# dnjulek/vapoursynth-zip

Measured on AMD Instinct MI355X. Metric: frames/sec at 4K YUV420P16: Bilateral, BoxBlur, SSIMULACRA2 on 1/2/4/8 MI355X, higher is better.
Workload: dtype u16; 1 GPU; vszip.BoxBlur hradius=vradius=13, 3840x2160 YUV420P16, splitmix64 noise, HBM-resident; parallelism=frame-parallel x1, arena_candidates=9

## Files before the change

### vapoursynth-zip_amd/csrc/boxblur_ct.hpp

```cpp
#pragma once
#include <cmath>
#include <cstdlib>
#include <utility>

#include "plane_table.hpp"

namespace {

#ifndef VSZIP_ST_AUX
#define VSZIP_ST_AUX 2
#endif
#ifndef VSZIP_LD_AUX
#define VSZIP_LD_AUX 0
#endif
#ifndef VSZIP_ST8_AUX
#define VSZIP_ST8_AUX 0
#endif
#ifndef VSZIP_ST16_AUX
#define VSZIP_ST16_AUX 2
#endif
constexpr int kStoreAux = VSZIP_ST_AUX, kLoadAux = VSZIP_LD_AUX, kStoreAux8 = VSZIP_ST8_AUX, kStoreAux16 = VSZIP_ST16_AUX;
typedef uint32_t U32x4 __attribute__((ext_vector_type(4)));
typedef uint32_t U32x2 __attribute__((ext_vector_type(2)));

constexpr int kMaxPlanes = 48;
constexpr int PX = 8;

struct BBPlane {
    const void *src;
    void *dst;
    int sstride, dstride;
    int w, h;
    int block0;
    int ntx;
    int nbands;
    int nperiods;
    int cx0;
};

struct BBParams {
    BBPlane p[kMaxPlanes];
    int nplanes;
    int band_rows;
    int nblocks;
};

constexpr int kRingMaxPlanes = 192;
constexpr int kRingMaxBlocks = 8192;
struct RingParams {
    BBPlane p[kRingMaxPlanes];
    int nplanes;
    int nblocks;
    uint8_t plane_of_block[kRingMaxBlocks];
};

__device__ __forceinline__ int ct_tap_row(int k, int i, int radius, int ih) {
    const int dist_from_bottom = ih - 1 - i;
    if (k < radius) return (i < radius - k) ? min(radius - k - i, ih - 1) : (i - radius + k);
    return (dist_from_bottom < k - radius) ? (i - min(k - radius - dist_from_bottom, i)) : (i - radius + k);
}

template <typename T>
struct Raw8;
template <>
struct Raw8<uint16_t> {
    uint4 q;
};
template <>
struct Raw8<uint8_t> {
    uint2 q;
};

__device__ __forceinline__ void unpack8(const Raw8<uint16_t> &r, uint32_t v[PX]) {
    v[0] = r.q.x & 0xffffu; v[1] = r.q.x >> 16;
    v[2] = r.q.y & 0xffffu; v[3] = r.q.y >> 16;
    v[4] = r.q.z & 0xffffu; v[5] = r.q.z >> 16;
    v[6] = r.q.w & 0xffffu; v[7] = r.q.w >> 16;
}

__device__ __forceinline__ void unpack8(const Raw8<uint8_t> &r, uint32_t v[PX]) {
    v[0] = r.q.x & 0xffu; v[1] = (r.q.x >> 8) & 0xffu; v[2] = (r.q.x >> 16) & 0xffu; v[3] = r.q.x >> 24;
    v[4] = r.q.y & 0xffu; v[5] = (r.q.y >> 8) & 0xffu; v[6] = (r.q.y >> 16) & 0xffu; v[7] = r.q.y >> 24;
}

__device__ __forceinline__ void pack8(const uint32_t v[PX], Raw8<uint16_t> &r) {
    r.q.x = v[0] | (v[1] << 16);
    r.q.y = v[2] | (v[3] << 16);
    r.q.z = v[4] | (v[5] << 16);
    r.q.w = v[6] | (v[7] << 16);
}

__device__ __forceinline__ void pack8(const uint32_t v[PX], Raw8<uint8_t> &r) {
    r.q.x = v[0] | (v[1] << 8) | (v[2] << 16) | (v[3] << 24);
    r.q.y = v[4] | (v[5] << 8) | (v[6] << 16) | (v[7] << 24);
}

template <typename T, int PXN>
struct RawN : Raw8<T> {};
template <>
struct RawN<uint8_t, 16> {
    uint4 q;
};
template <typename T>
__device__ __forceinline__ void unpackN(const RawN<T, 8> &r, uint32_t v[8]) {
    unpack8(static_cast<const Raw8<T> &>(r), v);
}
__device__ __forceinline__ void unpackN(const RawN<uint8_t, 16> &r, uint32_t v[16]) {
    const uint32_t dw[4] = {r.q.x, r.q.y, r.q.z, r.q.w};
#pragma unroll
    for (int k = 0; k < 16; ++k) v[k] = (dw[k >> 2] >> (8 * (k & 3))) & 0xffu;
}

__device__ __forceinline__ int mirror_col(int c, int w) {
    c = c < 0 ? -c - 1 : c;
    c = c >= w ? 2 * w - 1 - c : c;
    return min(max(c, 0), w - 1);
}

template <typename T>
__device__ __forceinline__ Raw8<T> load8(const T *row, int vx0, int w, bool fast) {
    Raw8<T> r;
    if (fast) {
        r.q = *reinterpret_cast<const decltype(r.q) *>(row + vx0);
    } else {
        uint32_t v[PX];
#pragma unroll
        for (int k = 0; k < PX; ++k) v[k] = row[mirror_col(vx0 + k, w)];
        pack8(v, r);
    }
    return r;
}

template <typename T>
__device__ __forceinline__ void store8(T *row, int x0, int w, bool fast, const uint32_t o[PX]);

template <>
__device__ __forceinline__ void store8<uint16_t>(uint16_t *row, int x0, int w, bool fast, const uint32_t o[PX]) {
    if (fast) {
        uint4 q;
        q.x = (o[0] & 0xffffu) | (o[1] << 16);
        q.y = (o[2] & 0xffffu) | (o[3] << 16);
        q.z = (o[4] & 0xffffu) | (o[5] << 16);
        q.w = (o[6] & 0xffffu) | (o[7] << 16);
        *reinterpret_cast<uint4 *>(row + x0) = q;
    } else {
#pragma unroll
        for (int k = 0; k < PX; ++k)
            if (x0 + k < w) row[x0 + k] = (uint16_t)o[k];
    }
}

template <>
__device__ __forceinline__ void store8<uint8_t>(uint8_t *row, int x0, int w, bool fast, const uint32_t o[PX]) {
    if (fast) {
        uint2 q;
        q.x = (o[0] & 0xffu) | ((o[1] & 0xffu) << 8) | ((o[2] & 0xffu) << 16) | (o[3] << 24);
        q.y = (o[4] & 0xffu) | ((o[5] & 0xffu) << 8) | ((o[6] & 0xffu) << 16) | (o[7] << 24);
        *reinterpret_cast<uint2 *>(row + x0) = q;
    } else {
#pragma unroll
        for (int k = 0; k < PX; ++k)
            if (x0 + k < w) row[x0 + k] = (uint8_t)o[k];
    }
}

template <int R>
struct CtGeom {
    static constexpr int K = 2 * R + 1;
    static constexpr int NE = (R + 1 + PX - 1) / PX;
    static constexpr int HL = NE * PX;
    static constexpr int HR = ((R + PX - 1) / PX) * PX;
    static constexpr int OUT_LANES = 64 - NE - HL / PX - HR / PX;
    static constexpr int TWO = OUT_LANES * PX;
};

__device__ __forceinline__ void wave_lds_fence() {
    __builtin_amdgcn_fence(__ATOMIC_RELEASE, "wavefront");
    __builtin_amdgcn_wave_barrier();
    __builtin_amdgcn_fence(__ATOMIC_ACQUIRE, "wavefront");
}

template <typename T, int R, bool DPP>
__global__ __launch_bounds__(64) void boxblur_ct_int_kernel(const BBParams prm) {
    using G = CtGeom<R>;
    constexpr uint32_t K = G::K;
    constexpr uint32_t MAGIC = (uint32_t)(((1ull << 32) + K - 1) / K);
    constexpr uint64_t INV = ((1ull << 32) + R) / K;
    constexpr uint32_t INV2 = (uint32_t)(INV >> 16);
    constexpr uint32_t INVLO = (uint32_t)(INV & 0xffffu);

    __shared__ __attribute__((aligned(16))) uint32_t P[64 * PX];

    const int b = blockIdx.x;
    const BBPlane pl = prm.p[vszip_find_plane(prm, b)];
    const int lb = b - pl.block0;
    const int tx = lb % pl.ntx;
    const int by = lb / pl.ntx;
    const int w = pl.w, h = pl.h;
    const int y0 = by * prm.band_rows;
    const int y1 = min(y0 + prm.band_rows, h);
    const T *src = static_cast<const T *>(pl.src);
    T *dst = static_cast<T *>(pl.dst);

    const int lane = threadIdx.x;
    const int X0 = tx * G::TWO;
    const int vx0 = lane < G::NE ? lane * PX : X0 - G::HL + (lane - G::NE) * PX;
    constexpr int VB = sizeof(T) * PX;
    const bool src_al = ((reinterpret_cast<uintptr_t>(src) | (uintptr_t)((size_t)pl.sstride * sizeof(T))) & (VB - 1)) == 0;
    const bool dst_al = ((reinterpret_cast<uintptr_t>(dst) | (uintptr_t)((size_t)pl.dstride * sizeof(T))) & (VB - 1)) == 0;
    const bool in_fast = src_al && vx0 >= 0 && vx0 + PX <= w;
    const bool is_out = lane >= G::NE + G::HL / PX && lane < G::NE + G::HL / PX + G::OUT_LANES && vx0 < w;
    const bool out_fast = dst_al && vx0 + PX <= w;

    uint32_t col[PX];
#pragma unroll
    for (int k = 0; k < PX; ++k) col[k] = 0;
#pragma unroll 1
    for (int k = 0; k < (int)K; ++k) {
        uint32_t v[PX];
        unpack8(load8<T>(src + (size_t)ct_tap_row(k, y0, R, h) * pl.sstride, vx0, w, in_fast), v);
#pragma unroll
        for (int j = 0; j < PX; ++j) col[j] += v[j];
    }

    const int ci = lane * PX;
#pragma unroll 1
    for (int i = y0; i < y1; ++i) {
        Raw8<T> an, sn;
        const bool more = i + 1 < y1;
        if (more) {
            const int n = i + 1;
            const int ar = (n + R < h) ? n + R : n - 1;
            const int sr = (n <= R) ? R - n + 1 : n - R - 1;
            an = load8<T>(src + (size_t)ar * pl.sstride, vx0, w, in_fast);
            sn = load8<T>(src + (size_t)sr * pl.sstride, vx0, w, in_fast);
        }

        uint32_t p[PX];
#pragma unroll
        for (int k = 0; k < PX; ++k) p[k] = __umulhi(col[k] + R, MAGIC);
#pragma unroll
        for (int k = 1; k < PX; ++k) p[k] += p[k - 1];
        const uint32_t incl = DPP ? wave_incl_scan_dpp(p[PX - 1]) : wave_incl_scan_shfl(p[PX - 1]);
        const uint32_t base = incl - p[PX - 1];
#pragma unroll
        for (int k = 0; k < PX; ++k) p[k] += base;
        *reinterpret_cast<uint4 *>(&P[ci]) = make_uint4(p[0], p[1], p[2], p[3]);
        *reinterpret_cast<uint4 *>(&P[ci + 4]) = make_uint4(p[4], p[5], p[6], p[7]);
        wave_lds_fence();

        if (is_out) {
            const uint32_t e0 = P[R] + P[R - 1];
            const uint32_t krow = 32768u + (uint32_t)(((uint64_t)e0 * INVLO) >> 16);
            uint32_t o[PX];
#pragma unroll
            for (int k = 0; k < PX; ++k) {
                const uint32_t e = P[ci + k + R] - P[ci + k - R - 1];
                o[k] = (uint32_t)(((uint64_t)e * INV2 + krow) >> 16);
            }
            store8<T>(dst + (size_t)i * pl.dstride, vx0, w, out_fast, o);
        }
        wave_lds_fence();

        if (more) {
            uint32_t a[PX], sb[PX];
            unpack8(an, a);
            unpack8(sn, sb);
#pragma unroll
            for (int k = 0; k < PX; ++k) col[k] += a[k] - sb[k];
        }
    }
}



template <int R, int SLOT_VGPRS = 4, int PXN = 8, int RV = R>
struct RingGeom {
    static constexpr int K = 2 * RV + 1;
    static constexpr int HL = ((R + 1 + PXN - 1) / PXN) * PXN;
    static constexpr int HR = ((R + PXN - 1) / PXN) * PXN;
#ifdef VSZIP_RING_OUT_LANES
    static constexpr int OUT_LANES = VSZIP_RING_OUT_LANES < 64 - HL / PXN - HR / PXN ? VSZIP_RING_OUT_LANES : 64 - HL / PXN - HR / PXN;
#else
    static constexpr int OUT_LANES = 64 - HL / PXN - HR / PXN;
#endif
    static constexpr int TWO = OUT_LANES * PXN;
    static constexpr int est_vgprs(int d) { return (2 * RV + 1 + d) * SLOT_VGPRS + (PXN == 16 ? 104 : 56); }
    static constexpr int tier(int v) { return v <= 128 ? 4 : (v <= 168 ? 3 : 2); }
    static constexpr int D3 = (2 * RV + 4) % 3 == 0 ? 3 : ((2 * RV + 6) % 3 == 0 ? 5 : 7);
#ifdef VSZIP_RING_D
    static constexpr int D = VSZIP_RING_D | 1;
    static constexpr int KL = (2 * RV + 1 + D) % 3 == 0 ? 3 : 2;
#else
    static constexpr bool SHALLOW = tier(est_vgprs(1)) > tier(est_vgprs(D3));
    static constexpr int D = SHALLOW ? 1 : D3;
    static constexpr int KL = SHALLOW ? 2 : 3;
#endif
    static constexpr int NR = 2 * RV + 1 + D;
#ifdef VSZIP_RING_WPE
    static constexpr int WPE = VSZIP_RING_WPE;
#else
    static constexpr int WPE = (SLOT_VGPRS == 2 && PXN == 8) ? (tier(est_vgprs(D)) > 3 ? 3 : tier(est_vgprs(D))) : tier(est_vgprs(D));
#endif
    static_assert(NR % KL == 0, "K-column ring must divide the period");
    static constexpr uint32_t MAGIC = K > 1 ? (uint32_t)(((1ull << 32) + K - 1) / K) : 0u;
};

template <typename T, int R, bool GENERAL, int PXN = 8, bool HONLY = false>
struct RingWave {
    static_assert(PXN == 8 || (PXN == 16 && sizeof(T) == 1 && !GENERAL), "16 pixels a lane: 8-bit planes, whole 16-pixel groups");
    static constexpr int RV = HONLY ? 0 : R;
    using G = RingGeom<R, (int)(sizeof(T) * PXN / 4), PXN, RV>;
    using RawT = RawN<T, PXN>;
    using Vec = decltype(RawT{}.q);
    static constexpr int NR = G::NR;
    static constexpr uint64_t INV = ((1ull << 32) + R) / (uint64_t)(2 * R + 1);
    static constexpr uint32_t INV2 = (uint32_t)(INV >> 16);

    RawT ring[NR];
    uint32_t col[PXN];
    uint32_t kcol;
    uint32_t kwgt;
    uint32_t kvo;
    uint32_t kn[G::KL], ko[G::KL];
    uint32_t kn_off, ko_off;
    uint32_t kr_prev;
    uint32_t *P;
    const char *srcb;
    char *dstb;
    uint32_t coff;
    uint32_t doff;
    uint32_t next_off;
    uint32_t out_off;
    uint32_t srow, drow;
    int w, h, lane, c0;
    bool rev, ld_ok, is_out, out_full;
    bool plain;
    __amdgpu_buffer_rsrc_t rs, rd;
    uint32_t sdoff;
    uint32_t psel;
    static constexpr uint32_t kOOB = 0xfffffff0u;

    __device__ __forceinline__ RawT fetch_off(uint32_t row_off) const {
        RawT t;
        if constexpr (sizeof(T) * PXN == 16) {
            const auto v = __builtin_amdgcn_raw_buffer_load_b128(rs, coff, row_off, sizeof(T) == 2 ? kLoadAux : 0);
            t.q = make_uint4(v[0], v[1], v[2], v[3]);
        } else {
            const auto v = __builtin_amdgcn_raw_buffer_load_b64(rs, coff, row_off, 0);
            t.q = make_uint2(v[0], v[1]);
        }
        return t;
    }
    __device__ __forceinline__ uint32_t fetch_px(uint32_t row_off) const {
        if constexpr (sizeof(T) == 2)
            return __builtin_amdgcn_raw_buffer_load_b16(rs, kvo, row_off, 0);
        else
            return __builtin_amdgcn_raw_buffer_load_b8(rs, kvo, row_off, 0);
    }
    __device__ __forceinline__ uint32_t krow_now() const {
        constexpr uint32_t INVLO = (uint32_t)(INV & 0xffffu);
        uint32_t v = __umul24(G::K > 1 ? __umulhi(kcol, G::MAGIC) : kcol, kwgt);
        v += (uint32_t)__builtin_amdgcn_update_dpp(0, (int)v, 0x111, 0xf, 0xf, false);
        v += (uint32_t)__builtin_amdgcn_update_dpp(0, (int)v, 0x112, 0xf, 0xf, false);
        v += (uint32_t)__builtin_amdgcn_update_dpp(0, (int)v, 0x114, 0xf, 0xf, false);
        v += (uint32_t)__builtin_amdgcn_update_dpp(0, (int)v, 0x118, 0xf, 0xf, false);
        uint32_t e0;
        if constexpr (R < 16) {
            e0 = (uint32_t)__builtin_amdgcn_readlane((int)v, 15);
        } else {
            v += (uint32_t)__builtin_amdgcn_update_dpp(0, (int)v, 0x142, 0xa, 0xf, false);
            e0 = (uint32_t)__builtin_amdgcn_readlane((int)v, 31);
        }
        return 32768u + (uint32_t)(((uint64_t)e0 * INVLO) >> 16);
    }

    __device__ __forceinline__ void fix_order(RawT &r) const {
        if constexpr (GENERAL) return;
        if constexpr (sizeof(T) * PXN == 16) {
            const uint4 o = r.q;
            r.q.x = __builtin_amdgcn_perm(o.w, o.x, psel);
            r.q.y = __builtin_amdgcn_perm(o.z, o.y, psel);
            r.q.z = __builtin_amdgcn_perm(o.y, o.z, psel);
            r.q.w = __builtin_amdgcn_perm(o.x, o.w, psel);
        } else {
            const uint2 o = r.q;
            r.q.x = __builtin_amdgcn_perm(o.y, o.x, psel);
            r.q.y = __builtin_amdgcn_perm(o.x, o.y, psel);
        }
    }
    __device__ __forceinline__ uint32_t row_off(int v) const {
        const int r = v < 0 ? -v : (v < h ? v : v - RV - 1);
        return (uint32_t)min(r, h - 1) * srow;
    }

    template <int J>
    __device__ __forceinline__ void fill(int y0) {
        ring[J] = fetch_off(row_off(y0 - RV + J));
    }
    template <int J>
    __device__ __forceinline__ void accum() {
        uint32_t v[PXN];
        fix_order(ring[J]);
        unpackN(ring[J], v);
#pragma unroll
        for (int k = 0; k < PXN; ++k) col[k] += v[k];
    }
    template <int... J>
    __device__ __forceinline__ void fill_all(int y0, std::integer_sequence<int, J...>) {
        (fill<(J + G::K) % NR>(y0), ...);
    }
    template <int... J>
    __device__ __forceinline__ void accum_all(std::integer_sequence<int, J...>) {
        (accum<J>(), ...);
    }

    static __device__ __forceinline__ int pidx(int c) { return (c & (PXN - 1)) * 64 + c / PXN; }

    __device__ __forceinline__ void window_sums(const uint32_t *Pb, uint32_t e[PXN]) const {
        if constexpr (!GENERAL) {
#pragma unroll
            for (int k = 0; k < PXN; ++k) {
                const int hi = k + R, lo = k - R - 1;
                const int hi_px = hi & (PXN - 1), hi_ln = hi / PXN;
                const int lo_px = lo & (PXN - 1), lo_ln = (lo - lo_px) / PXN;
                e[k] = Pb[hi_px * 64 + lane + hi_ln] - Pb[lo_px * 64 + lane + lo_ln];
            }
        } else {
            const int off = lane * PXN - c0;
            auto lds = [&](int idx) { return Pb[pidx(min(max(idx, 0), 64 * PXN - 1))]; };
            const uint32_t qw = lds(w - 1 + off);
#pragma unroll
            for (int k = 0; k < PXN; ++k) {
                const int x = c0 + k;
                const int lo = x - R - 1, ml = R - x - 1;
                uint32_t v = lds(min(x + R, w - 1) + off) + qw - lds(min(2 * w - 2 - x - R, w - 1) + off);
                v -= lo >= 0 ? lds(lo + off) : 0u;
                v += ml >= 0 ? lds(ml + off) : 0u;
                e[k] = v;
            }
        }
    }

    __device__ __forceinline__ void emit_row(const uint32_t e[PXN], uint32_t row_off_bytes, uint32_t kr, bool live) const {
        if constexpr (GENERAL) {
            if (!live || !is_out) return;
        }
        uint32_t t[PXN];
#pragma unroll
        for (int k = 0; k < PXN; ++k) t[k] = __umul24(e[k], INV2) + kr;
        if constexpr (!GENERAL) {
#ifdef VSZIP_DIAG_NO_STORE
            const uint32_t vo = (live && lane == 8) ? sdoff : kOOB;
#else
            const uint32_t vo = live ? sdoff : kOOB;
#endif
            if constexpr (sizeof(T) == 2) {
                U32x4 v;
                v.x = __builtin_amdgcn_perm(t[1], t[0], 0x07060302u);
                v.y = __builtin_amdgcn_perm(t[3], t[2], 0x07060302u);
                v.z = __builtin_amdgcn_perm(t[5], t[4], 0x07060302u);
                v.w = __builtin_amdgcn_perm(t[7], t[6], 0x07060302u);
                __builtin_amdgcn_raw_buffer_store_b128(v, rd, vo, row_off_bytes, kStoreAux);
            } else if constexpr (PXN == 16) {
                uint32_t dw[4];
#pragma unroll
                for (int g = 0; g < 4; ++g) {
                    const uint32_t a0 = __builtin_amdgcn_perm(t[4 * g + 1], t[4 * g], 0x0c0c0602u);
                    const uint32_t a1 = __builtin_amdgcn_perm(t[4 * g + 3], t[4 * g + 2], 0x0c0c0602u);
                    dw[g] = a0 | (a1 << 16);
                }
                U32x4 v;
                v.x = dw[0];
                v.y = dw[1];
                v.z = dw[2];
                v.w = dw[3];
                __builtin_amdgcn_raw_buffer_store_b128(v, rd, vo, row_off_bytes, kStoreAux16);
            } else {
                U32x2 v;
                const uint32_t a0 = __builtin_amdgcn_perm(t[1], t[0], 0x0c0c0602u);
                const uint32_t a1 = __builtin_amdgcn_perm(t[3], t[2], 0x0c0c0602u);
                const uint32_t a2 = __builtin_amdgcn_perm(t[5], t[4], 0x0c0c0602u);
                const uint32_t a3 = __builtin_amdgcn_perm(t[7], t[6], 0x0c0c0602u);
                v.x = a0 | (a1 << 16);
                v.y = a2 | (a3 << 16);
                __builtin_amdgcn_raw_buffer_store_b64(v, rd, vo, row_off_bytes, kStoreAux8);
            }
        } else {
            T *q = reinterpret_cast<T *>(dstb + (row_off_bytes + doff));
            if (out_full) {
                if constexpr (sizeof(T) == 2) {
                    uint4 v;
                    v.x = __builtin_amdgcn_perm(t[1], t[0], 0x07060302u);
                    v.y = __builtin_amdgcn_perm(t[3], t[2], 0x07060302u);
                    v.z = __builtin_amdgcn_perm(t[5], t[4], 0x07060302u);
                    v.w = __builtin_amdgcn_perm(t[7], t[6], 0x07060302u);
                    *reinterpret_cast<uint4 *>(q) = v;
                } else {
                    uint2 v;
                    const uint32_t a0 = __builtin_amdgcn_perm(t[1], t[0], 0x0c0c0602u);
                    const uint32_t a1 = __builtin_amdgcn_perm(t[3], t[2], 0x0c0c0602u);
                    const uint32_t a2 = __builtin_amdgcn_perm(t[5], t[4], 0x0c0c0602u);
                    const uint32_t a3 = __builtin_amdgcn_perm(t[7], t[6], 0x0c0c0602u);
                    v.x = a0 | (a1 << 16);
                    v.y = a2 | (a3 << 16);
                    *reinterpret_cast<uint2 *>(q) = v;
                }
            } else {
#pragma unroll
                for (int k = 0; k < PXN; ++k)
                    if (c0 + k < w) q[k] = (T)(t[k] >> 16);
            }
        }
    }

    template <int S>
    __device__ __forceinline__ void step(int i, int y0) {
        uint32_t *Pa = P + (S & 1) * (64 * PXN);
        const uint32_t *Pb = P + ((S & 1) ^ 1) * (64 * PXN);
        __builtin_amdgcn_sched_barrier(0);

        uint32_t e[PXN];
        const bool have_prev = S > 0 || i > y0;
#ifdef VSZIP_DIAG_NO_HORIZONTAL
#pragma unroll
        for (int k = 0; k < PXN; ++k) e[k] = col[k];
#else
        if (!GENERAL || have_prev) window_sums(Pb, e);
#endif

        uint32_t p[PXN];
#pragma unroll
        for (int k = 0; k < PXN; ++k) {
            if constexpr (G::K == 1) {
                p[k] = col[k];
            } else if constexpr (sizeof(T) == 1) {
                constexpr uint32_t M19 = (uint32_t)(((1u << 19) + G::K - 1) / G::K);
                static_assert((uint64_t)(255u * G::K + RV) * (M19 * G::K - (1u << 19)) < (1u << 19), "8-bit divide-by-k shortcut must be exact");
                p[k] = __umul24(col[k], M19) >> 19;
            } else {
                p[k] = __umulhi(col[k], G::MAGIC);
            }
        }
        if constexpr (GENERAL) {
            const uint32_t m = ld_ok ? 0xffffffffu : 0u;
#pragma unroll
            for (int k = 0; k < PXN; ++k) p[k] &= m;
        }
#ifdef VSZIP_DIAG_NO_HORIZONTAL
        (void)Pa;
        kr_prev += p[0] + p[7];
#else
#pragma unroll
        for (int k = 1; k < PXN; ++k) p[k] += p[k - 1];
        const uint32_t incl = wave_incl_scan_dpp(p[PXN - 1]);
        const uint32_t base = incl - p[PXN - 1];
#pragma unroll
        for (int k = 0; k < PXN; ++k) Pa[k * 64 + lane] = p[k] + base;
#endif

        {
            constexpr int E = (S + 1 + 2 * RV) % NR;
            uint32_t a[PXN], sb[PXN];
            fix_order(ring[E]);
            unpackN(ring[E], a);
            unpackN(ring[S], sb);
#pragma unroll
            for (int k = 0; k < PXN; ++k) col[k] += a[k] - sb[k];
#ifdef VSZIP_DIAG_NO_LOAD
            if (next_off == 0xffffffffu) ring[S] = fetch_off(next_off);
#else
            ring[S] = fetch_off(next_off);
#endif

        }
        const uint32_t kr_cur = krow_now();
        {
            constexpr int J = S % G::KL;
            kcol += kn[J] - ko[J];
#ifndef VSZIP_DIAG_NO_KCOL
            kn[J] = fetch_px(kn_off);
            ko[J] = fetch_px(ko_off);
#endif

        }

        emit_row(e, out_off, kr_prev, have_prev);
        out_off += have_prev ? drow : 0u;
        kr_prev = kr_cur;
        if (plain) {
            next_off += srow;
            kn_off += srow;
            ko_off += srow;
        } else {
            next_off = row_off(i + 2 + RV + G::D);
            kn_off = row_off(i + 2 + RV + G::KL);
            ko_off = row_off(i + 1 - RV + G::KL);
        }
#ifndef VSZIP_DIAG_NO_FENCE
        wave_lds_fence();
#endif
    }

    template <int... S>
    __device__ __forceinline__ void period(int i0, int y0, std::integer_sequence<int, S...>) {
        (step<S>(i0 + S, y0), ...);
    }
};

template <typename T, int R, bool GENERAL, int PXN = 8, bool HONLY = false>
__global__ __launch_bounds__(64, (GENERAL ? 2 : RingGeom<R, (int)(sizeof(T) * PXN / 4), PXN, (HONLY ? 0 : R)>::WPE)) void boxblur_ct_ring_kernel(const RingParams prm) {
    using W = RingWave<T, R, GENERAL, PXN, HONLY>;
    using G = typename W::G;
    constexpr int RV = W::RV;
    static_assert(G::NR % 2 == 0 && G::NR <= 64, "ring period must be even and fit a wave");
    __shared__ __attribute__((aligned(16))) uint32_t P[2 * 64 * PXN];

    const int chunk = (prm.nblocks + 7) >> 3;
    const int b = (int)(blockIdx.x & 7) * chunk + (int)(blockIdx.x >> 3);
    if (b >= prm.nblocks) return;
    const int pi = prm.plane_of_block[b];
    const BBPlane pl = prm.p[pi];
    const int lb = b - pl.block0;
    const int tx = lb % pl.ntx;
    const int by = lb / pl.ntx;
    const int p0 = (int)((long)by * pl.nperiods / pl.nbands);
    const int p1 = (int)((long)(by + 1) * pl.nperiods / pl.nbands);
    const int band_rows = (p1 - p0) * G::NR;
    const int y0 = min(p0 * G::NR, pl.h - band_rows);
    const int w = pl.w;

    W st;
    st.P = P;
    st.w = w;
    st.h = pl.h;
    st.srow = (uint32_t)pl.sstride * (uint32_t)sizeof(T);
    st.drow = (uint32_t)pl.dstride * (uint32_t)sizeof(T);
    st.srcb = static_cast<const char *>(pl.src);
    st.dstb = static_cast<char *>(pl.dst);
    const int lane = threadIdx.x;
    st.lane = lane;
    const int vc0 = pl.cx0 + tx * G::TWO - G::HL + lane * PXN;
    st.c0 = vc0;
    st.is_out = lane >= G::HL / PXN && lane < G::HL / PXN + G::OUT_LANES && vc0 < w;
    st.doff = (uint32_t)(max(vc0, 0) * (int)sizeof(T));
    st.out_full = vc0 + PXN <= w;
    if constexpr (!GENERAL) {
        int g = vc0;
        st.rev = false;
        if (vc0 < 0) {
            g = -vc0 - PXN;
            st.rev = true;
        } else if (vc0 >= w) {
            g = 2 * w - vc0 - PXN;
            st.rev = true;
        }
        g = min(max(g, 0), w - PXN);
        st.coff = (uint32_t)(g * (int)sizeof(T));
        st.ld_ok = true;
    } else {
        st.rev = false;
        st.ld_ok = vc0 >= 0 && vc0 < w;
        st.coff = (uint32_t)(min(max(vc0, 0), ((w - 1) / PXN) * PXN) * (int)sizeof(T));
    }

    st.psel = st.rev ? (sizeof(T) == 2 ? 0x05040706u : 0x04050607u) : 0x03020100u;
    st.sdoff = st.is_out ? st.doff : W::kOOB;
    st.rs = __builtin_amdgcn_make_buffer_rsrc(const_cast<void *>(pl.src), 0, (int)((uint32_t)pl.h * st.srow), 0x00020000);
    st.rd = __builtin_amdgcn_make_buffer_rsrc(pl.dst, 0, (int)((uint32_t)pl.h * st.drow), 0x00020000);
    st.plain = (y0 - RV >= 0) && (y0 + band_rows + RV + G::D + 2 < pl.h);

    st.fill_all(y0, std::make_integer_sequence<int, G::NR>{});
#pragma unroll
    for (int k = 0; k < PXN; ++k) st.col[k] = RV;
    st.accum_all(std::make_integer_sequence<int, (int)G::K>{});
    {
        const int kc = min(lane, R);
        st.kvo = (uint32_t)(kc * (int)sizeof(T));
        st.kwgt = lane < R ? 2u : (lane == R ? 1u : 0u);
        uint32_t acc = RV;
#pragma unroll
        for (int k = 0; k < (int)G::K; ++k) acc += st.fetch_px(st.row_off(y0 - RV + k));
        st.kcol = acc;
#pragma unroll
        for (int j = 0; j < G::KL; ++j) {
            st.kn[j] = st.fetch_px(st.row_off(y0 + j + 1 + RV));
            st.ko[j] = st.fetch_px(st.row_off(y0 + j - RV));
        }
        st.kn_off = st.row_off(y0 + G::KL + 1 + RV);
        st.ko_off = st.row_off(y0 + G::KL - RV);
        st.kr_prev = 0;
    }
    st.next_off = st.row_off(y0 + 1 + RV + G::D);
    st.out_off = (uint32_t)y0 * st.drow;

    const int y1 = y0 + band_rows;
#pragma unroll 1
    for (int i0 = y0; i0 < y1; i0 += G::NR) st.period(i0, y0, std::make_integer_sequence<int, G::NR>{});
    {
        uint32_t e[PXN];
        st.window_sums(P + 64 * PXN, e);
        st.emit_row(e, st.out_off, st.kr_prev, true);
    }
}


template <typename T, int R>
int launch_ct_int(vszip_ctx *ctx, const vszip_plane *planes, int nplanes) {
    using G = CtGeom<R>;
    int done = 0;
    while (done < nplanes) {
        BBParams prm;
        const int n = std::min(kMaxPlanes, nplanes - done);
        prm.nplanes = n;
        long total_px = 0;
        for (int i = 0; i < n; ++i) total_px += (long)planes[done + i].w * planes[done + i].h;
        int band = 64;
        while (band > 16 && total_px / ((long)G::TWO * band) < 4096) band >>= 1;
        prm.band_rows = band;
        int blocks = 0;
        for (int i = 0; i < n; ++i) {
            const vszip_plane &s = planes[done + i];
            BBPlane &d = prm.p[i];
            d.src = s.src;
            d.dst = s.dst;
            d.sstride = (int)s.src_stride;
            d.dstride = (int)s.dst_stride;
            d.w = s.w;
            d.h = s.h;
            d.block0 = blocks;
            d.ntx = (s.w + G::TWO - 1) / G::TWO;
            d.nbands = (s.h + band - 1) / band;
            blocks += d.ntx * d.nbands;
        }
        if (ctx->scan_mode == 1)
            hipLaunchKernelGGL((boxblur_ct_int_kernel<T, R, false>), dim3(blocks), dim3(64), 0, ctx->stream, prm);
        else
            hipLaunchKernelGGL((boxblur_ct_int_kernel<T, R, true>), dim3(blocks), dim3(64), 0, ctx->stream, prm);
        VSZIP_HIP_CHECK(ctx, hipGetLastError());
        done += n;
    }
    return VSZIP_OK;
}

struct RingSpan {
    int cx0, ntx;
};

template <typename T, int R, int PXN, bool HONLY = false>
int ring_plan(const vszip_plane *planes, const RingSpan *spans, int n, double *waves_ret) {
    using G = typename RingWave<T, R, false, PXN, HONLY>::G;
    struct Geo {
        int h, ntx, count;
    };
    std::vector<Geo> geos;
    for (int i = 0; i < n; ++i) {
        bool found = false;
        for (Geo &g : geos)
            if (g.h == planes[i].h && g.ntx == spans[i].ntx) {
                ++g.count;
                found = true;
                break;
            }
        if (!found) geos.push_back({planes[i].h, spans[i].ntx, 1});
    }
        auto bands_for = [](int h, int P, int target) { return std::max((h % G::NR != 0 && P >= 2) ? 2 : 1, (P + target / 2) / target); };
        const double halo_p = (double)(G::K - 1 + G::D) / G::NR;
        const double slots = 256.0 * 4 * G::WPE;
        double waves_out = 0;
        auto cost_for = [&](int target) {
            double work = 0, waves = 0, max_len = 0;
            for (const Geo &g : geos) {
                const int P = (g.h + G::NR - 1) / G::NR;
                const int nb = bands_for(g.h, P, target);
                const double ntx = (double)g.ntx * g.count;
                work += ntx * (P + nb * halo_p);
                waves += ntx * nb;
                max_len = std::max(max_len, (double)((P + nb - 1) / nb) + halo_p);
            }
            waves_out = waves;
            const double gens = std::ceil(waves / slots);
            const double eff = std::min(1.0, work / (slots * gens * max_len));
            return std::max(work / slots * (1.0 + 0.3 * (1.0 - eff)), 0.3 * max_len);
        };
        int target = 1;
        double best = cost_for(1);
        const double min_waves = std::min(0.6 * slots, waves_out);
        for (int t = 2; t <= 96; ++t) {
            const double c = cost_for(t);
            if (waves_out >= min_waves && c < best) {
                best = c;
                target = t;
            }
        }
        *waves_ret = (cost_for(target), waves_out);
        return target;
}


template <typename T, int R, int PXN, bool GEN, bool HONLY = false>
int launch_ct_ring_spans(vszip_ctx *ctx, const vszip_plane *all_planes, const RingSpan *all_spans, int nall) {
    using G = typename RingWave<T, R, false, PXN, HONLY>::G;
    std::vector<vszip_plane> planes_v;
    std::vector<RingSpan> spans_v;
    for (int i = 0; i < nall; ++i)
        if (all_spans[i].ntx > 0) {
            planes_v.push_back(all_planes[i]);
            spans_v.push_back(all_spans[i]);
        }
    const vszip_plane *planes = planes_v.data();
    const RingSpan *spans = spans_v.data();
    const int nplanes = (int)planes_v.size();
    int done = 0;
    while (done < nplanes) {
        RingParams prm;
        const int n = std::min(kRingMaxPlanes, nplanes - done);
        auto bands_for = [](int h, int P, int target) { return std::max((h % G::NR != 0 && P >= 2) ? 2 : 1, (P + target / 2) / target); };
        double waves_out = 0;
        int target = ring_plan<T, R, PXN, HONLY>(planes + done, spans + done, n, &waves_out);
        if (ctx->opt.ring_periods > 0) target = ctx->opt.ring_periods;
#ifdef VSZIP_RING_PERIODS_FIXED
        target = VSZIP_RING_PERIODS_FIXED;
#endif
#ifdef VSZIP_RING_PLAN_DEBUG
        fprintf(stderr, "ring plan PX%d GEN%d r=%d: n=%d target=%d waves=%.0f slots=%d NR=%d | plane0 %dx%d ntx=%d\n", PXN, (int)GEN, R, n, target, waves_out, 256 * 4 * G::WPE, G::NR,
                planes[done].w, planes[done].h, spans[done].ntx);
#endif
        VSZIP_HIP_CHECK(ctx, hipSetDevice(ctx->device));
        int blocks = 0, fit = n;
        for (int i = 0; i < n; ++i) {
            const vszip_plane &s = planes[done + i];
            BBPlane &d = prm.p[i];
            d.src = s.src;
            d.dst = s.dst;
            d.sstride = (int)s.src_stride;
            d.dstride = (int)s.dst_stride;
            d.w = s.w;
            d.h = s.h;
            d.nperiods = (s.h + G::NR - 1) / G::NR;
            d.nbands = bands_for(s.h, d.nperiods, target);
            d.ntx = spans[done + i].ntx;
            d.cx0 = spans[done + i].cx0;
            d.block0 = blocks;
            if (blocks + d.ntx * d.nbands > kRingMaxBlocks) {
                if (i == 0) return vszip_set_error(ctx, VSZIP_ERR_ARG, "BoxBlur: launch table overflow (%d blocks)", blocks + d.ntx * d.nbands);
                fit = i;
                break;
            }
            for (int k = 0; k < d.ntx * d.nbands; ++k) prm.plane_of_block[blocks + k] = (uint8_t)i;
            blocks += d.ntx * d.nbands;
        }
        prm.nplanes = fit;
        prm.nblocks = blocks;
        const dim3 grid(((blocks + 7) / 8) * 8);
        {
            vszip_probe_scope probe(ctx);
            hipLaunchKernelGGL((boxblur_ct_ring_kernel<T, R, GEN, PXN, HONLY>), grid, dim3(64), 0, ctx->stream, prm);
        }
        VSZIP_HIP_CHECK(ctx, hipGetLastError());
        done += fit;
    }
    return VSZIP_OK;
}

template <typename T>
bool ring_ok(const vszip_plane *planes, int nplanes) {
    constexpr uintptr_t VB = sizeof(T) * PX;
    for (int i = 0; i < nplanes; ++i) {
        const vszip_plane &p = planes[i];
        if ((reinterpret_cast<uintptr_t>(p.src) | reinterpret_cast<uintptr_t>(p.dst) | (uintptr_t)(p.src_stride * sizeof(T)) | (uintptr_t)(p.dst_stride * sizeof(T))) & (VB - 1)) return false;
        if (p.src_stride < ((p.w + PX - 1) / PX) * PX) return false;
        if (p.src_stride < 24) return false;
        if (p.h < 2 * 22 + 1 + 8) return false;
        if ((uint64_t)p.src_stride * p.h * sizeof(T) >= (1ull << 32) || (uint64_t)p.dst_stride * p.h * sizeof(T) >= (1ull << 32)) return false;
    }
    return true;
}

constexpr int kRing16MaxR = 19;
template <typename T, int R, bool HONLY = false>
bool ring16_ok(const vszip_ctx *ctx, const vszip_plane *planes, int nplanes) {
    if (sizeof(T) != 1 || ctx->opt.ct_u8_px8) return false;
    using G16 = RingGeom<R, 4, 16, (HONLY ? 0 : R)>;
    using G8 = RingGeom<R, 2, 8, (HONLY ? 0 : R)>;
    double px = 0, t16 = 0, t8 = 0;
    for (int i = 0; i < nplanes; ++i) {
        const vszip_plane &p = planes[i];
        if (p.w < 32) return false;
        if ((reinterpret_cast<uintptr_t>(p.src) | reinterpret_cast<uintptr_t>(p.dst) | (uintptr_t)p.src_stride | (uintptr_t)p.dst_stride) & 15) return false;
        px += (double)p.w * p.h;
        t16 += (double)((p.w + G16::TWO - 1) / G16::TWO) * G16::TWO * p.h;
        t8 += (double)((p.w + G8::TWO - 1) / G8::TWO) * G8::TWO * p.h;
    }
    if (R >= 8 && px / t16 < 0.93 * (px / t8)) return false;
    if (R >= 8) {
        const int n = std::min(nplanes, kRingMaxPlanes);
        std::vector<RingSpan> s16(n), s8(n);
        for (int i = 0; i < n; ++i) {
            s16[i] = {0, (planes[i].w + G16::TWO - 1) / G16::TWO};
            s8[i] = {0, (planes[i].w + G8::TWO - 1) / G8::TWO};
        }
        double w16 = 0, w8 = 0;
        ring_plan<T, R, 16, HONLY>(planes, s16.data(), n, &w16);
        ring_plan<T, R, 8, HONLY>(planes, s8.data(), n, &w8);
        const double f16 = w16 / (256.0 * 4 * G16::WPE), f8 = w8 / (256.0 * 4 * G8::WPE);
        if (f16 < 0.8 && f8 > f16 + 0.05) return false;
    }
    return true;
}

template <typename T, int R, int PXF, bool HONLY = false>
int run_ct_ring(vszip_ctx *ctx, const vszip_plane *planes, int nplanes) {
    using GF = typename RingWave<T, R, false, PXF, HONLY>::G;
    using GG = typename RingWave<T, R, true, 8, HONLY>::G;
    std::vector<RingSpan> fast(nplanes), rest(nplanes);
    bool any_rest = false, any_fast = false;
    for (int i = 0; i < nplanes; ++i) {
        const int w = planes[i].w;
        if (w % PXF == 0) {
            fast[i] = {0, (w + GF::TWO - 1) / GF::TWO};
            rest[i] = {0, 0};
        } else {
            const int room = w + GF::HL - 64 * PXF;
            const int nsafe = room >= 0 ? room / GF::TWO + 1 : 0;
            fast[i] = {0, nsafe};
            const int x = nsafe * GF::TWO;
            rest[i] = {x, (w - x + GG::TWO - 1) / GG::TWO};
        }
        any_fast = any_fast || fast[i].ntx > 0;
        any_rest = any_rest || rest[i].ntx > 0;
    }
    if (any_fast) {
        const int rc = launch_ct_ring_spans<T, R, PXF, false, HONLY>(ctx, planes, fast.data(), nplanes);
        if (rc != VSZIP_OK) return rc;
    }
    if (any_rest) return launch_ct_ring_spans<T, R, 8, true, HONLY>(ctx, planes, rest.data(), nplanes);
    return VSZIP_OK;
}

#ifdef VSZIP_DEV_R
#define VSZIP_R_ENABLED(R) ((R) == VSZIP_DEV_R)
#else
#define VSZIP_R_ENABLED(R) true
#endif

template <typename T, int R, int RLO>
struct CtIntDispatch {
    static int run(vszip_ctx *ctx, int r, const vszip_plane *planes, int nplanes) {
        if constexpr (VSZIP_R_ENABLED(R)) if (r == R) {
            if (ctx->scan_mode == 0 && ring_ok<T>(planes, nplanes)) {
                if constexpr (sizeof(T) == 1 && R <= kRing16MaxR) {
                    if (ring16_ok<T, R>(ctx, planes, nplanes)) return run_ct_ring<T, R, 16>(ctx, planes, nplanes);
                }
                return run_ct_ring<T, R, 8>(ctx, planes, nplanes);
            }
            return launch_ct_int<T, R>(ctx, planes, nplanes);
        }
        if constexpr (R > RLO)
            return CtIntDispatch<T, R - 1, RLO>::run(ctx, r, planes, nplanes);
        else
            return vszip_set_error(ctx, VSZIP_ERR_ARG, "BoxBlur: CT radius not built (development build?)");
    }
    static int run_h(vszip_ctx *ctx, int r, const vszip_plane *planes, int nplanes) {
        if constexpr (VSZIP_R_ENABLED(R)) if (r == R) {
            if (ctx->scan_mode != 0 || !ring_ok<T>(planes, nplanes)) return VSZIP_ERR_UNSUPPORTED;
            if constexpr (sizeof(T) == 1) {
                if (ring16_ok<T, R, true>(ctx, planes, nplanes)) return run_ct_ring<T, R, 16, true>(ctx, planes, nplanes);
            }
            return run_ct_ring<T, R, 8, true>(ctx, planes, nplanes);
        }
        if constexpr (R > RLO)
            return CtIntDispatch<T, R - 1, RLO>::run_h(ctx, r, planes, nplanes);
        else
            return VSZIP_ERR_UNSUPPORTED;
    }
};

}
```

### vapoursynth-zip_amd/csrc/common.hpp

```cpp
#pragma once
#include <hip/hip_runtime.h>

#include <cstdarg>
#include <cstdint>
#include <cstdio>
#include <mutex>
#include <string>
#include <vector>

#include "../../include/vszip_hip.h"

#define VSZIP_EXPORT extern "C" __attribute__((visibility("default")))

#if !defined(VSZIP_DEV_VARIANTS) &&                                                                                                              \
    (defined(VSZIP_XPSNR_TIMING_NOTEMP) || defined(VSZIP_XPSNR_TIMING_NOEDGE) || defined(VSZIP_SSIM_TIMING_NOF64) || defined(VSZIP_SSIM_TIMING_NOFETCH) || \
     defined(VSZIP_E3_DIAG_ONE_PASS) || defined(VSZIP_E3_DIAG_NO_DP) || defined(VSZIP_E3_DIAG_NO_BACKTRACK) || defined(VSZIP_DIAG_NO_KCOL) ||        \
     defined(VSZIP_DIAG_NO_FENCE) || defined(VSZIP_DIAG_NO_STORE) || defined(VSZIP_DIAG_NO_LOAD) || defined(VSZIP_DIAG_NO_HORIZONTAL))
#error "VSZIP_*_TIMING_* / VSZIP_*DIAG_* macros build kernels with wrong results: they need -DVSZIP_DEV_VARIANTS (tools/variant.sh)"
#endif

struct vszip_options {
#define VSZIP_OPT(field, env, def) int field = def;
#ifdef VSZIP_DEV_VARIANTS
#define VSZIP_DEV_OPT(field, env, def) int field = def;
#else
#define VSZIP_DEV_OPT(field, env, def) static constexpr int field = def;
#endif
#include "options.inc"
#undef VSZIP_OPT
#undef VSZIP_DEV_OPT
};

struct vszip_ctx {
    vszip_options opt;
    int device = 0;
    int num_cus = 0;
    hipStream_t stream = nullptr;
    bool own_stream = false;
    hipEvent_t ev0 = nullptr, ev1 = nullptr;
    hipStream_t aux_stream = nullptr;
    hipEvent_t aux_fork = nullptr, aux_join = nullptr;
    int aux_reserved = 0;
    hipStream_t side_stream = nullptr;
    hipEvent_t side_fork = nullptr, side_join = nullptr;
    std::string err;
    void *scratch = nullptr;
    size_t scratch_bytes = 0;
    void *scalars_dev = nullptr;
    void *scalars_host = nullptr;
    size_t scalars_bytes = 0;
    bool probe_on = false;
    std::vector<hipEvent_t> probe_events;
    size_t probe_used = 0;
    void *xpsnr_sums = nullptr;
    size_t xpsnr_sums_bytes = 0;
    bool xpsnr_clean = false;
    int &staging = opt.staging;
    char *stage = nullptr;
    size_t stage_bytes = 0, stage_used = 0;
    struct PendingOut {
        void *dst;
        size_t dpitch;
        const char *src;
        size_t wb, rows;
    };
    std::vector<PendingOut> pending_out;
    void *minmax_pred = nullptr;
    size_t minmax_pred_planes = 0;
    std::vector<uint64_t> minmax_sig;
    std::vector<uint64_t> minmax_used;
    uint64_t minmax_tick = 0;
    int minmax_predicted = 0;
    int minmax_fallbacks = 0;
    void *chain_buf = nullptr;
    size_t chain_bytes = 0;
    void *ssim_lut = nullptr;
    int &scan_mode = opt.scan_mode;
    hipEvent_t probe_ev0 = nullptr, probe_ev1 = nullptr;
};

int vszip_set_error(vszip_ctx *ctx, int code, const char *fmt, ...);
int vszip_ensure_scratch(vszip_ctx *ctx, size_t bytes);
hipError_t vszip_hip_malloc(vszip_ctx *ctx, void **p, size_t bytes);
int vszip_ensure_scalars(vszip_ctx *ctx, size_t bytes);
void vszip_ssim_release(vszip_ctx *ctx);
void vszip_chain_release(vszip_ctx *ctx);
void vszip_planestats_release(vszip_ctx *ctx);
void vszip_bilateral_forget_lut(const void *dptr);
void vszip_probe_mark(vszip_ctx *ctx);
void vszip_aux_register(vszip_ctx *ctx);

struct vszip_probe_scope {
    vszip_ctx *c;
    explicit vszip_probe_scope(vszip_ctx *ctx) : c(ctx) { if (c->probe_on) vszip_probe_mark(c); }
    ~vszip_probe_scope() { if (c->probe_on) vszip_probe_mark(c); }
};

#define VSZIP_HIP_CHECK(ctx, call)                                                              \
    do {                                                                                        \
        hipError_t e_ = (call);                                                                 \
        if (e_ != hipSuccess)                                                                   \
            return vszip_set_error((ctx), VSZIP_ERR_HIP, "%s failed: %s", #call, hipGetErrorString(e_)); \
    } while (0)

static inline int vszip_dtype_size(int dt) {
    switch (dt) {
        case VSZIP_U8: return 1;
        case VSZIP_U16: return 2;
        case VSZIP_F16: return 2;
        case VSZIP_F32: return 4;
        case VSZIP_U32: return 4;
    }
    return 0;
}

#if defined(__HIPCC__)

__device__ __forceinline__ uint32_t wave_incl_scan_dpp(uint32_t v) {
    v += (uint32_t)__builtin_amdgcn_update_dpp(0, (int)v, 0x111, 0xf, 0xf, false);
    v += (uint32_t)__builtin_amdgcn_update_dpp(0, (int)v, 0x112, 0xf, 0xf, false);
    v += (uint32_t)__builtin_amdgcn_update_dpp(0, (int)v, 0x114, 0xf, 0xf, false);
    v += (uint32_t)__builtin_amdgcn_update_dpp(0, (int)v, 0x118, 0xf, 0xf, false);
    v += (uint32_t)__builtin_amdgcn_update_dpp(0, (int)v, 0x142, 0xa, 0xf, false);
    v += (uint32_t)__builtin_amdgcn_update_dpp(0, (int)v, 0x143, 0xc, 0xf, false);
    return v;
}

__device__ __forceinline__ uint32_t wave_incl_scan_shfl(uint32_t v) {
    const int lane = threadIdx.x & 63;
#pragma unroll
    for (int d = 1; d < 64; d <<= 1) {
        const uint32_t o = __shfl_up(v, d, 64);
        if (lane >= d) v += o;
    }
    return v;
}

__device__ __forceinline__ void vszip_wave_fence() {
    __builtin_amdgcn_fence(__ATOMIC_RELEASE, "wavefront");
    __builtin_amdgcn_wave_barrier();
    __builtin_amdgcn_fence(__ATOMIC_ACQUIRE, "wavefront");
}

template <typename T>
__device__ __forceinline__ T wave_reduce_sum(T v) {
#pragma unroll
    for (int d = 32; d >= 1; d >>= 1) v += __shfl_down(v, d, 64);
    return v;
}

#endif
```

Before: 112,400 frames/s.

## Batch border K-row computation across wave lane groups to amortize scans

Replaces the per-row serial K-row computation (a column sum over lanes 0..R plus a DPP scan and readlane every row) with batched evaluation. The wave is split into KB groups of 64/KB lanes, so several consecutive rows' K values come from one DPP scan and are read out with one readlane each. Column sums are carried between groups with ds_bpermute, and the pixel fetches are issued once per batch instead of twice per row. The warmup placement is also made configurable per instantiation to tune overlap with the ring fill. In exchange it adds bpermute latency and lane-index bookkeeping, and makes the R < KGW constraint stricter.

```diff
diff --git a/vapoursynth-zip_amd/csrc/boxblur_ct.hpp b/vapoursynth-zip_amd/csrc/boxblur_ct.hpp
--- a/vapoursynth-zip_amd/csrc/boxblur_ct.hpp
+++ b/vapoursynth-zip_amd/csrc/boxblur_ct.hpp
@@ -290,11 +290,9 @@
     static constexpr int D3 = (2 * RV + 4) % 3 == 0 ? 3 : ((2 * RV + 6) % 3 == 0 ? 5 : 7);
 #ifdef VSZIP_RING_D
     static constexpr int D = VSZIP_RING_D | 1;
-    static constexpr int KL = (2 * RV + 1 + D) % 3 == 0 ? 3 : 2;
 #else
     static constexpr bool SHALLOW = tier(est_vgprs(1)) > tier(est_vgprs(D3));
     static constexpr int D = SHALLOW ? 1 : D3;
-    static constexpr int KL = SHALLOW ? 2 : 3;
 #endif
     static constexpr int NR = 2 * RV + 1 + D;
 #ifdef VSZIP_RING_WPE
@@ -302,7 +300,9 @@
 #else
     static constexpr int WPE = (SLOT_VGPRS == 2 && PXN == 8) ? (tier(est_vgprs(D)) > 3 ? 3 : tier(est_vgprs(D))) : tier(est_vgprs(D));
 #endif
-    static_assert(NR % KL == 0, "K-column ring must divide the period");
+    static constexpr int KB = (R < 16 && NR % 4 == 0) ? 4 : 2;
+    static constexpr int KGW = 64 / KB;
+    static_assert(NR % KB == 0 && R < KGW, "K_row batches must tile the period and hold columns 0..r");
     static constexpr uint32_t MAGIC = K > 1 ? (uint32_t)(((1ull << 32) + K - 1) / K) : 0u;
 };
 
@@ -319,11 +319,11 @@
 
     RawT ring[NR];
     uint32_t col[PXN];
-    uint32_t kcol;
-    uint32_t kwgt;
+    uint32_t kcv;
     uint32_t kvo;
-    uint32_t kn[G::KL], ko[G::KL];
-    uint32_t kn_off, ko_off;
+    uint32_t kpe, kpl;
+    uint32_t kd, kb, kcarry;
+    uint32_t kr[G::KB];
     uint32_t kr_prev;
     uint32_t *P;
     const char *srcb;
@@ -352,27 +352,84 @@
         }
         return t;
     }
-    __device__ __forceinline__ uint32_t fetch_px(uint32_t row_off) const {
+    __device__ __forceinline__ uint32_t fetch_px(uint32_t vo, uint32_t row_off) const {
         if constexpr (sizeof(T) == 2)
-            return __builtin_amdgcn_raw_buffer_load_b16(rs, kvo, row_off, 0);
+            return __builtin_amdgcn_raw_buffer_load_b16(rs, vo, row_off, 0);
         else
-            return __builtin_amdgcn_raw_buffer_load_b8(rs, kvo, row_off, 0);
-    }
-    __device__ __forceinline__ uint32_t krow_now() const {
+            return __builtin_amdgcn_raw_buffer_load_b8(rs, vo, row_off, 0);
+    }
+    __device__ __forceinline__ int lane_now() const {
+        int l = lane;
+        asm volatile("" : "+v"(l));
+        return l;
+    }
+    __device__ __forceinline__ uint32_t krow_vo(int v0) const {
+        const int l = lane_now();
+        const int c = l & (G::KGW - 1);
+        return c <= R ? row_off(v0 + (int)((uint32_t)l / G::KGW)) + (uint32_t)(c * (int)sizeof(T)) : kOOB;
+    }
+    __device__ __forceinline__ uint32_t krow_batch() const {
         constexpr uint32_t INVLO = (uint32_t)(INV & 0xffffu);
-        uint32_t v = __umul24(G::K > 1 ? __umulhi(kcol, G::MAGIC) : kcol, kwgt);
+#ifdef VSZIP_DIAG_CONST_KROW
+        return 32768u + INVLO;
+#endif
+        const uint32_t kwgt = (uint32_t)min(max(R + 1 - (lane_now() & (G::KGW - 1)), 0), 2);
+        uint32_t v = __umul24(G::K > 1 ? __umulhi(kcv, G::MAGIC) : kcv, kwgt);
         v += (uint32_t)__builtin_amdgcn_update_dpp(0, (int)v, 0x111, 0xf, 0xf, false);
         v += (uint32_t)__builtin_amdgcn_update_dpp(0, (int)v, 0x112, 0xf, 0xf, false);
         v += (uint32_t)__builtin_amdgcn_update_dpp(0, (int)v, 0x114, 0xf, 0xf, false);
         v += (uint32_t)__builtin_amdgcn_update_dpp(0, (int)v, 0x118, 0xf, 0xf, false);
-        uint32_t e0;
-        if constexpr (R < 16) {
-            e0 = (uint32_t)__builtin_amdgcn_readlane((int)v, 15);
-        } else {
-            v += (uint32_t)__builtin_amdgcn_update_dpp(0, (int)v, 0x142, 0xa, 0xf, false);
-            e0 = (uint32_t)__builtin_amdgcn_readlane((int)v, 31);
-        }
-        return 32768u + (uint32_t)(((uint64_t)e0 * INVLO) >> 16);
+        if constexpr (G::KGW == 32) v += (uint32_t)__builtin_amdgcn_update_dpp(0, (int)v, 0x142, 0xa, 0xf, false);
+        return 32768u + (uint32_t)(((uint64_t)(v & 0xffffffu) * INVLO) >> 16);
+    }
+    __device__ __forceinline__ void krow_warmup(int y0) {
+        constexpr int KB = G::KB, GW = G::KGW;
+        const int kc = lane & (GW - 1);
+        kvo = kc <= R ? (uint32_t)(kc * (int)sizeof(T)) + (uint32_t)(lane / GW) * srow : kOOB;
+        uint32_t acc = RV;
+#pragma unroll
+        for (int k = 0; k < (int)G::K; ++k) acc += fetch_px(krow_vo(y0 - RV + k), 0);
+        kcv = acc;
+        kpe = fetch_px(krow_vo(y0 + KB + RV), 0);
+        kpl = fetch_px(krow_vo(y0 + KB - 1 - RV), 0);
+        kd = kb = kcarry = 0;
+#pragma unroll
+        for (int j = 0; j < KB; ++j) kr[j] = 0;
+        kr_prev = 0;
+    }
+    template <int PH>
+    __device__ __forceinline__ void krow_step(int i) {
+        constexpr int KB = G::KB, GW = G::KGW;
+        if constexpr (PH == 0) {
+            const uint32_t kv = krow_batch();
+#pragma unroll
+            for (int j = 0; j < KB; ++j) kr[j] = (uint32_t)__builtin_amdgcn_readlane((int)kv, j * GW + GW - 1);
+            kd = kpe - kpl;
+            kb = (uint32_t)__builtin_amdgcn_ds_bpermute((lane - GW) * 4, (int)kd);
+            kcarry = (uint32_t)__builtin_amdgcn_ds_bpermute((lane_now() | ((KB - 1) * GW)) * 4, (int)kcv);
+        } else if constexpr (PH == 1) {
+            kd += lane >= GW ? kb : 0u;
+            if constexpr (KB == 2)
+                kcv = kcarry + kd;
+            else
+                kb = (uint32_t)__builtin_amdgcn_ds_bpermute((lane - 2 * GW) * 4, (int)kd);
+        } else if constexpr (PH == 2) {
+            kcv = kcarry + kd + (lane >= 2 * GW ? kb : 0u);
+        }
+        if constexpr (PH == KB - 1) {
+            const int vl0 = i - PH + 2 * KB - 1 - RV;
+            uint32_t ve = kvo, vl = kvo, se = (uint32_t)(vl0 + 2 * RV + 1) * srow, sl = (uint32_t)vl0 * srow;
+            if (vl0 < 0 || vl0 + 2 * RV + KB >= h) {
+                ve = krow_vo(vl0 + 2 * RV + 1);
+                vl = krow_vo(vl0);
+                se = 0;
+                sl = 0;
+            }
+#ifndef VSZIP_DIAG_NO_KCOL
+            kpe = fetch_px(ve, se);
+            kpl = fetch_px(vl, sl);
+#endif
+        }
     }
 
     __device__ __forceinline__ void fix_order(RawT &r) const {
@@ -562,7 +619,9 @@
         {
             constexpr int E = (S + 1 + 2 * RV) % NR;
             uint32_t a[PXN], sb[PXN];
+#ifndef VSZIP_DIAG_NO_FIXORDER
             fix_order(ring[E]);
+#endif
             unpackN(ring[E], a);
             unpackN(ring[S], sb);
 #pragma unroll
@@ -574,28 +633,16 @@
 #endif
 
         }
-        const uint32_t kr_cur = krow_now();
-        {
-            constexpr int J = S % G::KL;
-            kcol += kn[J] - ko[J];
-#ifndef VSZIP_DIAG_NO_KCOL
-            kn[J] = fetch_px(kn_off);
-            ko[J] = fetch_px(ko_off);
-#endif
-
-        }
+        krow_step<S % G::KB>(i);
+        const uint32_t kr_cur = kr[S % G::KB];
 
         emit_row(e, out_off, kr_prev, have_prev);
         out_off += have_prev ? drow : 0u;
         kr_prev = kr_cur;
         if (plain) {
             next_off += srow;
-            kn_off += srow;
-            ko_off += srow;
         } else {
             next_off = row_off(i + 2 + RV + G::D);
-            kn_off = row_off(i + 2 + RV + G::KL);
-            ko_off = row_off(i + 1 - RV + G::KL);
         }
 #ifndef VSZIP_DIAG_NO_FENCE
         wave_lds_fence();
@@ -607,6 +654,14 @@
         (step<S>(i0 + S, y0), ...);
     }
 };
+
+template <typename T, int R, bool GENERAL, int PXN, bool HONLY>
+constexpr int ring_k_warmup_pos() {
+    if constexpr (!HONLY && sizeof(T) == 2 && GENERAL && R == 17) return 2;
+    if constexpr (!HONLY && sizeof(T) == 2 && GENERAL && R == 19) return 1;
+    if constexpr (!HONLY && sizeof(T) == 1 && !GENERAL && PXN == 8 && R == 22) return 1;
+    return GENERAL || (sizeof(T) == 1 && PXN == 8) ? 0 : 2;
+}
 
 template <typename T, int R, bool GENERAL, int PXN = 8, bool HONLY = false>
 __global__ __launch_bounds__(64, (GENERAL ? 2 : RingGeom<R, (int)(sizeof(T) * PXN / 4), PXN, (HONLY ? 0 : R)>::WPE)) void boxblur_ct_ring_kernel(const RingParams prm) {
@@ -670,27 +725,14 @@
     st.rd = __builtin_amdgcn_make_buffer_rsrc(pl.dst, 0, (int)((uint32_t)pl.h * st.drow), 0x00020000);
     st.plain = (y0 - RV >= 0) && (y0 + band_rows + RV + G::D + 2 < pl.h);
 
+    constexpr int K_POS = ring_k_warmup_pos<T, R, GENERAL, PXN, HONLY>();
+    if constexpr (K_POS == 0) st.krow_warmup(y0);
     st.fill_all(y0, std::make_integer_sequence<int, G::NR>{});
+    if constexpr (K_POS == 1) st.krow_warmup(y0);
 #pragma unroll
     for (int k = 0; k < PXN; ++k) st.col[k] = RV;
     st.accum_all(std::make_integer_sequence<int, (int)G::K>{});
-    {
-        const int kc = min(lane, R);
-        st.kvo = (uint32_t)(kc * (int)sizeof(T));
-        st.kwgt = lane < R ? 2u : (lane == R ? 1u : 0u);
-        uint32_t acc = RV;
-#pragma unroll
-        for (int k = 0; k < (int)G::K; ++k) acc += st.fetch_px(st.row_off(y0 - RV + k));
-        st.kcol = acc;
-#pragma unroll
-        for (int j = 0; j < G::KL; ++j) {
-            st.kn[j] = st.fetch_px(st.row_off(y0 + j + 1 + RV));
-            st.ko[j] = st.fetch_px(st.row_off(y0 + j - RV));
-        }
-        st.kn_off = st.row_off(y0 + G::KL + 1 + RV);
-        st.ko_off = st.row_off(y0 + G::KL - RV);
-        st.kr_prev = 0;
-    }
+    if constexpr (K_POS == 2) st.krow_warmup(y0);
     st.next_off = st.row_off(y0 + 1 + RV + G::D);
     st.out_off = (uint32_t)y0 * st.drow;
 
diff --git a/vapoursynth-zip_amd/csrc/common.hpp b/vapoursynth-zip_amd/csrc/common.hpp
--- a/vapoursynth-zip_amd/csrc/common.hpp
+++ b/vapoursynth-zip_amd/csrc/common.hpp
@@ -15,6 +15,7 @@
 #if !defined(VSZIP_DEV_VARIANTS) &&                                                                                                              \
     (defined(VSZIP_XPSNR_TIMING_NOTEMP) || defined(VSZIP_XPSNR_TIMING_NOEDGE) || defined(VSZIP_SSIM_TIMING_NOF64) || defined(VSZIP_SSIM_TIMING_NOFETCH) || \
      defined(VSZIP_E3_DIAG_ONE_PASS) || defined(VSZIP_E3_DIAG_NO_DP) || defined(VSZIP_E3_DIAG_NO_BACKTRACK) || defined(VSZIP_DIAG_NO_KCOL) ||        \
+     defined(VSZIP_DIAG_CONST_KROW) || defined(VSZIP_DIAG_NO_FIXORDER) ||                                                                            \
      defined(VSZIP_DIAG_NO_FENCE) || defined(VSZIP_DIAG_NO_STORE) || defined(VSZIP_DIAG_NO_LOAD) || defined(VSZIP_DIAG_NO_HORIZONTAL))
 #error "VSZIP_*_TIMING_* / VSZIP_*DIAG_* macros build kernels with wrong results: they need -DVSZIP_DEV_VARIANTS (tools/variant.sh)"
 #endif
```

Result: slower. 110,400 frames/s (-1.7%).
